# robert80203/HuPR-A-Benchmark-for-Human-Pose-Estimation-Using-Millimeter-Wave-Radar

Measured on AMD Instinct MI355X. Metric: radar frames/sec (FFT->heatmap fwd+bwd), higher is better.
Workload: dtype bf16

## Files before the change

### hupr-a-benchmark-for-human-pose-estimation-using-millimeter-wave-radar_amd/csrc/conv_halo256m_bf16.hip

```cpp
#include "conv_halo.h"

namespace hupr {

typedef float f32x4c __attribute__((ext_vector_type(4)));

template <int TD, int TH, int TW, int KD, int NCOT = 0, int NWN = 2, int KC = 64>
__global__ __launch_bounds__(512) void hupr_k_conv_halo256m_bf16(HaloArgs p) {
    constexpr int LDK = KC, BN = 32 * NWN, TS = KC == 64 ? 3 : 9, C8 = KC / 8, L2C8 = KC == 64 ? 3 : 2;
    static_assert(KC == 64 || (KC == 32 && KD == 3 && NWN == 2 && NCOT == 0), "32-channel rows: 3 x 3 x 3 taps, 64 output channels per tile");
    constexpr int HD = TD + KD - 1, HH = TH + 2, HW = TW + 2;
    static_assert(TD * TH * TW == 64 * (8 / NWN) && TH % 8 == 0 && TW % 8 == 0 && (KD == 1 || KD == 3) && (NWN == 2 || NCOT == 0),
                  "256 (512) voxels per tile, 8 x 8 per wave");
    constexpr int NVOX = HD * HH * HW;
    constexpr int T = 9 * KD, NSTAGE = KC == 64 ? 3 * KD : KD, NTAP = KC == 64 ? 6 : 9;
    constexpr bool FULLD = NWN == 1;
    constexpr int NVOXL = FULLD ? TD * HH * HW : NVOX, VOX0 = FULLD ? HH * HW : 0;
    constexpr int NH = (NVOXL * C8 + 511) / 512;
    constexpr int Y0 = NH < NTAP - 1 ? NH : NTAP - 1, Y1 = NH - (NTAP - 1) < 0 ? 0 : (NH - (NTAP - 1) > NTAP ? NTAP : NH - (NTAP - 1)),
                  Y2 = NH - (2 * NTAP - 1) < 0 ? 0 : (NH - (2 * NTAP - 1) > NTAP ? NTAP : NH - (2 * NTAP - 1));
    static_assert(NH <= NTAP * NSTAGE - 1 && NH <= 3 * NTAP - 1, "halo items must all be issued in front of the item's last barrier (and within three stages)");
    __shared__ __attribute__((aligned(16))) __bf16 Hs[(KC == 32 ? 2 : 1) * NVOX * LDK];
    __shared__ __attribute__((aligned(16))) __bf16 Bs[2][TS][BN * LDK];
    constexpr bool STATS = NCOT > 0 && KD == 3;
    constexpr bool SINGLE = STATS && TD == 2;
    f32x4c ssum[STATS ? NCOT : 1][2], ssq[STATS ? NCOT : 1][2];
    if constexpr (!SINGLE) {
#pragma unroll
        for (int ct = 0; ct < (STATS ? NCOT : 1); ++ct)
#pragma unroll
            for (int cg = 0; cg < 2; ++cg) { ssum[ct][cg] = (f32x4c){0.f, 0.f, 0.f, 0.f}; ssq[ct][cg] = (f32x4c){0.f, 0.f, 0.f, 0.f}; }
    }

    const int tid = threadIdx.x, lane = tid & 63, wave = tid >> 6;
    if (wave >= 4) __builtin_amdgcn_s_setprio(1);
    const int wm = NWN == 2 ? wave >> 1 : wave, wn = NWN == 2 ? wave & 1 : 0;
    constexpr int NBX = TW / 8, NBY = TH / 8;
    const int xw0 = 8 * (wm % NBX), yw0 = 8 * ((wm / NBX) % NBY), dzw = wm / (NBX * NBY);
    const int idx = lane & 15, kq = lane >> 4, yy = idx >> 3, wx = idx & 7;
    const int n_tiles = p.Bn * p.nd * p.nh * p.nw * p.n_co_tiles;

    const int wrow_ = NWN == 2 ? 8 * wave + (lane >> 3) : ((8 * wave + (lane >> 3)) & 31);
    const int wsrc_lane = (wrow_ * T * p.Ci + (((lane & 7) ^ (wrow_ >> 1)) & 7) * 8) * 2 +
                          (NWN == 2 ? 0 : (wave >> 2) * (3 * p.Ci * 2));
    constexpr int NDMA = NWN == 2 ? TS : 2, DMA_TAPS = NWN == 2 ? 1 : 2;
    const int wrow32_ = 16 * (wave & 3) + (lane >> 2);
    const int wsrc32_lane = (wrow32_ * T * p.Ci + (((lane & 3) ^ (((wrow32_ >> 3) & 1) << 1)) & 3) * 8) * 2;
    const u32x4 wrs = {(unsigned)(unsigned long)p.wp, (unsigned)((unsigned long)p.wp >> 32) & 0xffffu,
                       (unsigned)((long)p.Co * T * p.Ci * 2), 0x00020000u};
    const unsigned bs_lds = (unsigned)(unsigned long)(__attribute__((address_space(3))) void*)&Bs[0][0][0];
    const unsigned wdst_wave = __builtin_amdgcn_readfirstlane(bs_lds + wave * 1024);
#define HUPR_W_DMA(COT_, CH_, S_, PAR_)                                                                             \
    if constexpr (KC == 32) {                                                                                       \
        _Pragma("unroll") for (int j = 0; j < 5; ++j) {                                                             \
            if (j < 4 || wave < 4) {                                                                                \
                const int t9_ = 2 * j + (wave >> 2);                                  \
                const int wb32_ = (((COT_) * BN * T + (S_) * 9 + (t9_ % 3) * 3 + t9_ / 3) * p.Ci + (CH_) * KC) * 2 + wsrc32_lane; \
                unsigned keep_;                                                                                     \
                asm volatile("s_mov_b32 %0, m0\n\ts_mov_b32 m0, %1\n\ts_nop 0\n\tbuffer_load_dwordx4 %2, %3, 0 offen lds\n\t" \
                             "s_mov_b32 m0, %0"                                                                     \
                             : "=&s"(keep_)                                                                         \
                             : "s"(wdst_wave + (PAR_) * TS * (BN * LDK * 2) + j * 8192), "v"(wb32_), "s"(wrs)       \
                             : "memory");                                                                           \
            }                                                                                                       \
        }                                                                                                           \
    } else {                                                                                                        \
        const int wbase_ = (((COT_) * BN * T + ((S_) / 3) * 9 + ((S_) % 3)) * p.Ci + (CH_) * KC) * 2 + wsrc_lane;   \
        _Pragma("unroll") for (int j = 0; j < NDMA; ++j) {                                                          \
            if (NWN == 2 || j == 0 || wave < 4) {                                                                   \
                unsigned keep_;                                                                                     \
                asm volatile("s_mov_b32 %0, m0\n\ts_mov_b32 m0, %1\n\ts_nop 0\n\tbuffer_load_dwordx4 %2, %3, 0 offen lds\n\t" \
                             "s_mov_b32 m0, %0"                                                                     \
                             : "=&s"(keep_)                                                                         \
                             : "s"(NWN == 2 ? wdst_wave + ((PAR_) * TS + j) * (BN * LDK * 2)                        \
                                            : wdst_wave + (PAR_) * TS * (BN * LDK * 2) + j * 8192),                 \
                               "v"(NWN == 2 ? wbase_ + j * (3 * p.Ci * 2) : wbase_ + j * DMA_TAPS * (3 * p.Ci * 2)), "s"(wrs) \
                             : "memory");                                                                           \
            }                                                                                                       \
        }                                                                                                           \
    }

    u32x4 vb[NH];
    const __amdgpu_buffer_rsrc_t xrs = __builtin_amdgcn_make_buffer_rsrc(
        const_cast<void*>(p.x), 0, (int)((long)p.Bn * p.D * p.H * p.W * p.in_ld * 2), 0x00020000);
#define HUPR_HALO_ISSUE_ITEM(u, COND_, B_, D0_, H0_, W0_, C0_)                                                     \
    {                                                                                                               \
        const int it = tid + (u) * 512;                                                                             \
        const int vox = it >> L2C8, c8 = it & (C8 - 1);                                                             \
        const int hx = vox % HW;                                                                                    \
        const int t_ = vox / HW;                                                                                    \
        const int hy = t_ % HH, hz = t_ / HH;                                                                       \
        const int d = (D0_) + hz - (FULLD ? 0 : KD / 2), h = (H0_) + hy - 1, w = (W0_) + hx - 1;                    \
        const bool ok = (COND_) && it < NVOXL * C8 && (unsigned)d < (unsigned)p.D && (unsigned)h < (unsigned)p.H && \
                        (unsigned)w < (unsigned)p.W;                                                                \
        const int off = (((((B_) * p.D + d) * p.H + h) * p.W + w) * p.in_ld + (C0_) + c8 * 8) * 2;                  \
        const auto ld_ = __builtin_amdgcn_raw_buffer_load_b128(xrs, ok ? off : 0x7ffffff0, 0, 0);                  \
        vb[u] = (u32x4){ld_[0], ld_[1], ld_[2], ld_[3]};                                                            \
    }
#define HUPR_HALO_COMMIT()                                                                                          \
    _Pragma("unroll") for (int u = 0; u < NH; ++u) {                                                                \
        const int it = tid + u * 512;                                                                               \
        if (it < NVOXL * C8) {                                                                                      \
            const int vox = it >> L2C8, c8 = it & (C8 - 1);                                                         \
            const int hx = vox % HW;                                                                                \
            const int key_ = KC == 64 ? (((hx >> 1) & 3) << 1) : ((((vox / HW) % HH) & 1) << 1);                    \
            *reinterpret_cast<u32x4*>(&Hs[(vox + VOX0) * LDK + ((c8 ^ key_) << 3)]) = vb[u];                        \
        }                                                                                                           \
    }

    struct Pos { int cot, twi, thi, tdi, b, ch; };
    const int n_chunks = p.Ci / KC;
    const int per_wg = (n_tiles + gridDim.x - 1) / gridDim.x;
    const int wg_rank = (int)((blockIdx.x & 7) * (gridDim.x >> 3) + (blockIdx.x >> 3));
    const int t_begin = wg_rank * per_wg, t_end = min(n_tiles, t_begin + per_wg);
    if (STATS && p.stats) {
        if (t_begin >= t_end) {
            for (int c = tid; c < 2 * p.Co; c += 512) p.stats[(long)blockIdx.x * 2 * p.Co + c] = 0.0;
        }
    }
    if (t_begin >= t_end) return;
    Pos cur;
    {
        cur.cot = t_begin % p.n_co_tiles;
        int st = t_begin / p.n_co_tiles;
        cur.twi = st % p.nw; st /= p.nw;
        cur.thi = st % p.nh; st /= p.nh;
        cur.tdi = st % p.nd;
        cur.b = st / p.nd;
        cur.ch = 0;
    }
    const int n_items = (t_end - t_begin) * n_chunks;
    const int cot0 = cur.cot;

    int woff[2][2];
#pragma unroll
    for (int cg = 0; cg < 2; ++cg)
#pragma unroll
        for (int kk = 0; kk < 2; ++kk) {
            const int n = 32 * wn + 16 * cg + idx;
            woff[cg][kk] = KC == 64 ? n * LDK + (((4 * kk + kq) ^ ((n >> 1) & 7)) << 3) : n * LDK + ((kq ^ (((n >> 3) & 1) << 1)) << 3);
        }
    const int xlane = ((dzw * HH + yw0 + yy) * HW + xw0 + wx) * LDK;
#define HUPR_HALO_COMMIT1(u, HW_)                                                                                   \
    {                                                                                                               \
        const int it = tid + (u) * 512;                                                                             \
        if (it < NVOXL * C8) {                                                                                      \
            const int vox = it >> L2C8, c8 = it & (C8 - 1);                                                         \
            const int key_ = (((vox / HW) % HH) & 1) << 1;                                                          \
            *reinterpret_cast<u32x4*>(&Hs[(HW_) + (vox + VOX0) * LDK + ((c8 ^ key_) << 3)]) = vb[u];                \
        }                                                                                                           \
    }
#define HUPR_XF(ST_, RHO_, KK_)                                                                                     \
    (KC == 64 ? *reinterpret_cast<const bf16x8*>(&Hs[xlane + ((((ST_) / 3) * HH + (RHO_)) * HW + ((ST_) % 3)) * LDK + \
                    (((4 * (KK_) + kq) ^ ((((xw0 + wx + ((ST_) % 3)) >> 1) & 3) << 1)) << 3)])                      \
              : *reinterpret_cast<const bf16x8*>(&Hs[hrd + xlane + (((ST_) * HH + (RHO_)) * HW + (KK_)) * LDK +     \
                    ((kq ^ (((yy + (RHO_)) & 1) << 1)) << 3)]))
#define HUPR_WF(BUF_, KY_, CG_, KK_)                                                                                \
    (KC == 64 ? *reinterpret_cast<const bf16x8*>(&Bs[BUF_][KY_][woff[CG_][KK_]])                                    \
              : *reinterpret_cast<const bf16x8*>(&Bs[BUF_][3 * (KK_) + (KY_)][woff[CG_][0]]))

    f32x4c c[4][2];
    unsigned accP[4][2][2];
    __bf16* pP = nullptr;
    bool pend = false;
    constexpr bool RESPF = !STATS && TD != 2 && NWN == 2;
    const bool res_pf = RESPF && p.res != nullptr && (p.res_ld & 3) == 0 && !p.no_res_prefetch;
    constexpr bool BIASPF = KC == 32;
    const bool defer = (!p.bias || BIASPF) && (!p.res || res_pf) && (p.Co & 7) == 0 && (p.out_ld & 7) == 0;
    float biasv[BIASPF ? 2 : 1][4];
    bf16x4 resv[4][2];
    constexpr int NB = KC == 64 ? 2 : 3;
    bf16x8 xq[NB][4], x8, wq[NB][2];
#define HUPR_LOAD_TAP(ST_, TAU_, BUF_, WX_)                                                                         \
    {                                                                                                               \
        constexpr int kk_ = (TAU_) / 3, ky_ = (TAU_) % 3;                                                           \
        if ((WX_) & 1) {                                                                                            \
            wq[(TAU_) % NB][0] = HUPR_WF(BUF_, ky_, 0, kk_);                                                        \
            wq[(TAU_) % NB][1] = HUPR_WF(BUF_, ky_, 1, kk_);                                                        \
        }                                                                                                           \
        if ((WX_) & 2) {                                                                                            \
            if (ky_ == 0) { _Pragma("unroll") for (int vg = 0; vg < 4; ++vg) xq[kk_ % NB][vg] = HUPR_XF(ST_, 2 * vg, kk_); } \
            else if (ky_ == 1) { _Pragma("unroll") for (int vg = 0; vg < 4; ++vg) xq[(kk_ + 1) % NB][vg] = HUPR_XF(ST_, 2 * vg + 1, kk_); } \
            else { x8 = HUPR_XF(ST_, 8, kk_); }                                                                     \
        }                                                                                                           \
    }
#define HUPR_VMCNT_LGKM0(N_) __builtin_amdgcn_s_waitcnt(0x0070 | ((N_) & 15) | (((N_) >> 4) << 14))

    if constexpr (FULLD) {
        for (int i = tid; i < 2 * HH * HW * C8; i += 512) {
            const int pl = i / (HH * HW * C8), r = i - pl * (HH * HW * C8);
            *reinterpret_cast<u32x4*>(&Hs[pl * (HD - 1) * HH * HW * LDK + r * 8]) = (u32x4){0u, 0u, 0u, 0u};
        }
    }
    HUPR_W_DMA(cur.cot, cur.ch, 0, 0)
    HUPR_W_DMA(cur.cot, cur.ch, 1, 1)
#pragma unroll
    for (int u = 0; u < NH; ++u) HUPR_HALO_ISSUE_ITEM(u, true, cur.b, cur.tdi * TD, cur.thi * TH, cur.twi * TW, cur.ch * KC)
    [[maybe_unused]] int hrd = 0;
    if constexpr (KC == 32) {
#pragma unroll
        for (int u = 0; u < NH; ++u) HUPR_HALO_COMMIT1(u, 0)
    } else {
        HUPR_HALO_COMMIT()
    }
    __builtin_amdgcn_s_waitcnt(0x0F70);
    __syncthreads();
    HUPR_LOAD_TAP(0, 0, 0, 3)

    int g = 0;
    for (int q = 0; q < n_items; ++q) {
        const int b = cur.b, d0 = cur.tdi * TD, h0 = cur.thi * TH, w0 = cur.twi * TW, n0 = cur.cot * BN;
        const bool first_chunk = cur.ch == 0, last_chunk = cur.ch == n_chunks - 1;
        Pos nxt = cur;
        if (++nxt.ch == n_chunks) {
            nxt.ch = 0;
            if (++nxt.cot == p.n_co_tiles) {
                nxt.cot = 0;
                if (++nxt.twi == p.nw) {
                    nxt.twi = 0;
                    if (++nxt.thi == p.nh) {
                        nxt.thi = 0;
                        if (++nxt.tdi == p.nd) { nxt.tdi = 0; ++nxt.b; }
                    }
                }
            }
        }
        const bool has_next = q + 1 < n_items;
        if constexpr (KC == 32) hrd = (q & 1) * (NVOX * LDK);
        [[maybe_unused]] const int hwr = NVOX * LDK - hrd;
        if (first_chunk) {
#pragma unroll
            for (int vg = 0; vg < 4; ++vg)
#pragma unroll
                for (int cg = 0; cg < 2; ++cg) c[vg][cg] = (f32x4c){0.f, 0.f, 0.f, 0.f};
            if constexpr (BIASPF) {
                if (p.bias && defer) {
#pragma unroll
                    for (int cg = 0; cg < 2; ++cg)
#pragma unroll
                        for (int r = 0; r < 4; ++r) biasv[cg][r] = p.bias[n0 + 32 * wn + 16 * cg + 4 * kq + r];
                }
            }
        }
#pragma unroll
        for (int st_ = 0; st_ < NSTAGE; ++st_) {
            const int par = (g + st_) & 1;
#pragma unroll
            for (int tau = 0; tau < NTAP; ++tau) {
                const int kk = tau / 3, ky = tau % 3;
                if (tau == NTAP - 1) {
                    if (st_ == 0) { if (pend) { HUPR_VMCNT_LGKM0(Y0 + 4); } else { HUPR_VMCNT_LGKM0(Y0); } }
                    else if (st_ == 1) { HUPR_VMCNT_LGKM0(Y1); }
                    else if (st_ == 2) { HUPR_VMCNT_LGKM0(Y2); }
                    else { HUPR_VMCNT_LGKM0(0); }
                    __syncthreads();
                    if (st_ + 2 < NSTAGE) { HUPR_W_DMA(cur.cot, cur.ch, st_ + 2, par) }
                    else if (has_next) { HUPR_W_DMA(nxt.cot, nxt.ch, st_ + 2 - NSTAGE, par) }
                    if (KC == 64 && st_ == NSTAGE - 1 && has_next) { HUPR_HALO_COMMIT() }
                }
                if (tau == 0) { HUPR_LOAD_TAP(st_, 1, par, 3) }
                else if (tau == 1) { HUPR_LOAD_TAP(st_, 2, par, 3) }
                else if (tau == 2) { HUPR_LOAD_TAP(st_, 3, par, 3) }
                else if (tau == 3) { HUPR_LOAD_TAP(st_, 4, par, 3) }
                else if (tau == 4) { HUPR_LOAD_TAP(st_, 5, par, 3) }
                else if (NTAP == 9 && tau == 5) { if constexpr (NTAP == 9) { HUPR_LOAD_TAP(st_, 6, par, 3) } }
                else if (NTAP == 9 && tau == 6) { if constexpr (NTAP == 9) { HUPR_LOAD_TAP(st_, 7, par, 3) } }
                else if (NTAP == 9 && tau == 7) { if constexpr (NTAP == 9) { HUPR_LOAD_TAP(st_, 8, par, 3) } }
                else if (st_ + 1 < NSTAGE) { HUPR_LOAD_TAP((st_ + 1) % NSTAGE, 0, par ^ 1, 3) }
                else if (has_next) {
                    if constexpr (KC == 32) { const int hrd = hwr; HUPR_LOAD_TAP(0, 0, par ^ 1, 3) }
                    else { HUPR_LOAD_TAP(0, 0, par ^ 1, 1) }
                }
#pragma unroll
                for (int vg = 0; vg < 4; ++vg) {
                    const bf16x8 xf = ky == 0 ? xq[kk % NB][vg] : (ky == 1 ? xq[(kk + 1) % NB][vg] : (vg < 3 ? xq[kk % NB][vg + 1] : x8));
                    c[vg][0] = __builtin_amdgcn_mfma_f32_16x16x32_bf16(wq[tau % NB][0], xf, c[vg][0], 0, 0, 0);
                    c[vg][1] = __builtin_amdgcn_mfma_f32_16x16x32_bf16(wq[tau % NB][1], xf, c[vg][1], 0, 0, 0);
                }
                if (st_ == 0 && pend && tau < 4) {
                    const auto r0 = __builtin_amdgcn_permlane16_swap(accP[tau][0][0], accP[tau][1][0], false, false);
                    const auto r1 = __builtin_amdgcn_permlane16_swap(accP[tau][0][1], accP[tau][1][1], false, false);
                    *reinterpret_cast<u32x4*>(pP + (long)(2 * tau * p.W) * p.out_ld) = (u32x4){r0[0], r1[0], r0[1], r1[1]};
                }
                if (RESPF && st_ == NSTAGE - 1 && tau == 0) {
                    if (res_pf && last_chunk && defer) {
                        const long mr = (((long)b * p.D + d0 + dzw) * p.H + h0 + yw0 + yy) * p.W + w0 + xw0 + wx;
                        const int chr = n0 + 32 * wn + 4 * kq;
#pragma unroll
                        for (int vg = 0; vg < 4; ++vg)
#pragma unroll
                            for (int cg = 0; cg < 2; ++cg)
                                resv[vg][cg] = *reinterpret_cast<const bf16x4*>(static_cast<const __bf16*>(p.res) + (mr + 2 * vg * p.W) * p.res_ld +
                                                                                chr + 16 * cg);
                    }
                }
                if constexpr (KC == 32) {
                    if (st_ == NSTAGE - 1 && tau < NH && has_next) { HUPR_HALO_COMMIT1(tau, hwr) }
                }
                if (NTAP * st_ + tau < NH) {
                    HUPR_HALO_ISSUE_ITEM(NTAP * st_ + tau, has_next, nxt.b, nxt.tdi * TD, nxt.thi * TH, nxt.twi * TW, nxt.ch * KC)
                }
                __builtin_amdgcn_sched_group_barrier(0x100, 1, 0);
                __builtin_amdgcn_sched_group_barrier(0x008, 2, 0);
                __builtin_amdgcn_sched_group_barrier(0x100, 1, 0);
                __builtin_amdgcn_sched_group_barrier(0x008, 2, 0);
#pragma unroll
                for (int i_ = 0; i_ < 4; ++i_) {
                    __builtin_amdgcn_sched_group_barrier(0x100, 1, 0);
                    __builtin_amdgcn_sched_group_barrier(0x008, 1, 0);
                }
                __builtin_amdgcn_sched_barrier(0);
            }
            if (st_ == 0) pend = false;
        }
        g += NSTAGE;
        if (last_chunk) {
            const long m0 = (((long)b * p.D + d0 + dzw) * p.H + h0 + yw0 + yy) * p.W + w0 + xw0 + wx;
            const int ch0 = n0 + 32 * wn + 4 * kq;
            typedef __bf16 bf16x2 __attribute__((ext_vector_type(2)));
            if (defer && has_next) {
                if constexpr (BIASPF) {
                    if (p.bias) {
#pragma unroll
                        for (int vg = 0; vg < 4; ++vg)
#pragma unroll
                            for (int cg = 0; cg < 2; ++cg)
#pragma unroll
                                for (int r = 0; r < 4; ++r) c[vg][cg][r] += biasv[cg][r];
                    }
                }
                if (RESPF && res_pf) {
#pragma unroll
                    for (int vg = 0; vg < 4; ++vg)
#pragma unroll
                        for (int cg = 0; cg < 2; ++cg)
#pragma unroll
                            for (int r = 0; r < 4; ++r) c[vg][cg][r] += (float)resv[vg][cg][r];
                }
#pragma unroll
                for (int vg = 0; vg < 4; ++vg)
#pragma unroll
                    for (int cg = 0; cg < 2; ++cg) {
                        const bf16x2 lo = {(__bf16)c[vg][cg][0], (__bf16)c[vg][cg][1]}, hi = {(__bf16)c[vg][cg][2], (__bf16)c[vg][cg][3]};
                        accP[vg][cg][0] = __builtin_bit_cast(unsigned, lo);
                        accP[vg][cg][1] = __builtin_bit_cast(unsigned, hi);
                    }
                pP = static_cast<__bf16*>(p.y) + m0 * p.out_ld + n0 + 32 * wn + ((kq & 1) ? 16 + 4 * (kq - 1) : 4 * kq);
                pend = true;
            } else {
#pragma unroll
                for (int vg = 0; vg < 4; ++vg)
#pragma unroll
                    for (int cg = 0; cg < 2; ++cg) {
                        const long m = m0 + 2 * vg * p.W;
                        const int ch = ch0 + 16 * cg;
                        if (ch < p.Co) {
                            f32x4n v = {c[vg][cg][0], c[vg][cg][1], c[vg][cg][2], c[vg][cg][3]};
                            if (p.bias) v += (f32x4n){p.bias[ch], p.bias[ch + 1], p.bias[ch + 2], p.bias[ch + 3]};
                            if (p.res) {
                                const bf16x4 rv = *reinterpret_cast<const bf16x4*>(static_cast<const __bf16*>(p.res) + m * p.res_ld + ch);
                                v += (f32x4n){(float)rv[0], (float)rv[1], (float)rv[2], (float)rv[3]};
                            }
                            const bf16x4 o = {(__bf16)v[0], (__bf16)v[1], (__bf16)v[2], (__bf16)v[3]};
                            *reinterpret_cast<bf16x4*>(static_cast<__bf16*>(p.y) + m * p.out_ld + ch) = o;
                        }
                    }
            }
            if (STATS && p.stats) {
                int li = cur.cot - cot0;
                li += li < 0 ? p.n_co_tiles : 0;
                if constexpr (SINGLE) {
#pragma unroll
                    for (int cg = 0; cg < 2; ++cg) {
                        f32x4c sv = {0.f, 0.f, 0.f, 0.f}, qv = sv;
#pragma unroll
                        for (int vg = 0; vg < 4; ++vg)
#pragma unroll
                            for (int r = 0; r < 4; ++r) {
                                const float a = (float)(__bf16)c[vg][cg][r];
                                sv[r] += a;
                                qv[r] = fmaf(a, a, qv[r]);
                            }
                        ssum[0][cg] = sv;
                        ssq[0][cg] = qv;
                    }
                } else {
#pragma unroll
                    for (int ct = 0; ct < NCOT; ++ct)
                        if (NCOT == 1 || li == ct) {
#pragma unroll
                            for (int cg = 0; cg < 2; ++cg)
#pragma unroll
                                for (int vg = 0; vg < 4; ++vg)
#pragma unroll
                                    for (int r = 0; r < 4; ++r) {
                                        const float a = (float)(__bf16)c[vg][cg][r];
                                        ssum[ct][cg][r] += a;
                                        ssq[ct][cg][r] = fmaf(a, a, ssq[ct][cg][r]);
                                    }
                        }
                }
            }
        }
        if (KC == 64 && has_next) {
            __syncthreads();
            HUPR_LOAD_TAP(0, 0, g & 1, 2)
        }
        cur = nxt;
    }
    if (STATS && p.stats) {
        static_assert(NVOX * LDK * 2 >= 8 * 64 * 16 * 4, "the halo image must hold the reduction scratch");
        float (*St)[64][16] = reinterpret_cast<float (*)[64][16]>(Hs);
#pragma unroll
        for (int ct = 0; ct < NCOT; ++ct) {
            __syncthreads();
#pragma unroll
            for (int cg = 0; cg < 2; ++cg) {
                *reinterpret_cast<f32x4c*>(&St[wave][lane][4 * cg]) = ssum[ct][cg];
                *reinterpret_cast<f32x4c*>(&St[wave][lane][8 + 4 * cg]) = ssq[ct][cg];
            }
            __syncthreads();
            if (tid < 2 * BN) {
                const int k = tid >> 6, ch = tid & 63;
                const int wn_ = ch >> 5, cg = (ch >> 4) & 1, kq_ = (ch >> 2) & 3, r = ch & 3;
                double t = 0.0;
#pragma unroll
                for (int wm_ = 0; wm_ < 4; ++wm_)
#pragma unroll
                    for (int i = 0; i < 16; ++i) t += (double)St[2 * wm_ + wn_][16 * kq_ + i][8 * k + 4 * cg + r];
                p.stats[(long)blockIdx.x * 2 * p.Co + k * p.Co + 64 * ((cot0 + ct) % p.n_co_tiles) + ch] = t;
            }
        }
        if (tid < 2 * BN) {
            const int k = tid >> 6, ch = tid & 63;
            for (int ct = NCOT; ct < p.n_co_tiles; ++ct)
                p.stats[(long)blockIdx.x * 2 * p.Co + k * p.Co + 64 * ((cot0 + ct) % p.n_co_tiles) + ch] = 0.0;
        }
    }
#undef HUPR_W_DMA
#undef HUPR_HALO_ISSUE_ITEM
#undef HUPR_HALO_COMMIT
#undef HUPR_HALO_COMMIT1
#undef HUPR_XF
#undef HUPR_WF
#undef HUPR_LOAD_TAP
#undef HUPR_VMCNT_LGKM0
}

void launch_conv_halo256(const HaloArgs& a, int route, hipStream_t s) {
    const dim3 grid(kHalo256Grid), wg(512);
    switch (route) {
    case kRouteCi32: HUPR_LAUNCH((hupr_k_conv_halo256m_bf16<4, 8, 8, 3, 0, 2, 32>), grid, wg, 0, s, a); break;
    case kRouteCo32: HUPR_LAUNCH((hupr_k_conv_halo256m_bf16<8, 8, 8, 3, 0, 1>), grid, wg, 0, s, a); break;
    case kRoute1x16x16: HUPR_LAUNCH((hupr_k_conv_halo256m_bf16<1, 16, 16, 1>), grid, wg, 0, s, a); break;
    case kRouteStats4x8x8One: HUPR_LAUNCH((hupr_k_conv_halo256m_bf16<4, 8, 8, 3, 1>), grid, wg, 0, s, a); break;
    case kRouteStats4x8x8Two: HUPR_LAUNCH((hupr_k_conv_halo256m_bf16<4, 8, 8, 3, 2>), grid, wg, 0, s, a); break;
    case kRouteStats2x8x16: HUPR_LAUNCH((hupr_k_conv_halo256m_bf16<2, 8, 16, 3, 1>), grid, wg, 0, s, a); break;
    case kRoute4x8x8: HUPR_LAUNCH((hupr_k_conv_halo256m_bf16<4, 8, 8, 3>), grid, wg, 0, s, a); break;
    case kRoute2x8x16: HUPR_LAUNCH((hupr_k_conv_halo256m_bf16<2, 8, 16, 3>), grid, wg, 0, s, a); break;
    }
}

static int g_halo_tiles = 31;
void set_halo_tiles(int mask) { g_halo_tiles = mask & 31; }

static bool offsets_fit(const HaloArgs& a, int Bn) { return (long)Bn * a.D * a.H * a.W * a.in_ld * 2 < 0x7ffffff0L; }

bool conv_halo256_supported(const HaloArgs& a, int Bn, bool abf) {
    if (!abf || !(g_halo_tiles & 1)) return false;
    if (a.kd != 3 || a.D % 4 != 0 || a.H % 8 != 0 || a.W % 8 != 0 || a.Ci % 64 != 0 || a.Co % 64 != 0) return false;
    const long tiles = (long)Bn * (a.D / 4) * (a.H / 8) * (a.W / 8) * (a.Co / 64);
    if (tiles >= (1L << 31) || tiles < 256) return false;
    return offsets_fit(a, Bn);
}

bool conv_halo256_stats_ok(const HaloArgs& a, int Bn) {
    if (a.kd != 3 || a.Ci % 64 != 0 || a.Co % 64 != 0 || !offsets_fit(a, Bn)) return false;
    const int n = a.Co / 64;
    if (a.D % 4 == 0) {
        if (!conv_halo256_supported(a, Bn, true)) return false;
        if (n == 1) return true;
        const long tiles = (long)Bn * (a.D / 4) * (a.H / 8) * (a.W / 8) * n;
        const long per_wg = (tiles + kHalo256Grid - 1) / kHalo256Grid;
        return n <= 2 || per_wg == 1;
    }
    if (!(g_halo_tiles & 2) || a.D % 2 != 0 || a.H % 8 != 0 || a.W % 16 != 0) return false;
    return (long)Bn * (a.D / 2) * (a.H / 8) * (a.W / 16) * n == 256;
}

int conv_halo256_route(HaloArgs& a, int Bn, bool abf) {
    if (!abf || !offsets_fit(a, Bn)) return 0;
    if (a.Ci == 32) {
        if (!(g_halo_tiles & 16) || a.kd != 3 || a.D % 4 != 0 || a.H % 8 != 0 || a.W % 8 != 0 || a.Co % 64 != 0 || a.stats ||
            (a.in_ld & 7) || (long)a.Co * 27 * a.Ci * 2 >= 0x7ffffff0L)
            return 0;
        a.n_co_tiles = a.Co / 64;
        a.TD = 4; a.log2TW = 3;
        a.nd = a.D / 4; a.nh = a.H / 8; a.nw = a.W / 8;
        const long tiles_ = (long)Bn * a.nd * a.nh * a.nw * a.n_co_tiles;
        if (tiles_ < 256 || tiles_ >= (1L << 31)) return 0;
        return kRouteCi32;
    }
    if (a.Ci % 64 != 0) return 0;
    if (a.Co == 32) {
        if (!(g_halo_tiles & 8) || a.kd != 3 || a.D != 8 || a.H % 8 != 0 || a.W % 8 != 0 || a.stats || (a.out_ld & 7)) return 0;
        a.n_co_tiles = 1;
        a.TD = 8; a.log2TW = 3;
        a.nd = a.D / 8; a.nh = a.H / 8; a.nw = a.W / 8;
        const long tiles32 = (long)Bn * a.nd * a.nh * a.nw;
        if (tiles32 < 256 || tiles32 >= (1L << 31)) return 0;
        return kRouteCo32;
    }
    if (a.Co % 64 != 0) return 0;
    a.n_co_tiles = a.Co / 64;
    if (a.kd == 3 && a.D % 4 == 0) {
        if (!conv_halo256_supported(a, Bn, abf)) return 0;
        a.TD = 4; a.log2TW = 3;
        a.nd = a.D / 4; a.nh = a.H / 8; a.nw = a.W / 8;
    } else if (a.kd == 3) {
        if (!(g_halo_tiles & 2) || a.D % 2 != 0 || a.H % 8 != 0 || a.W % 16 != 0) return 0;
        a.TD = 2; a.log2TW = 4;
        a.nd = a.D / 2; a.nh = a.H / 8; a.nw = a.W / 16;
    } else {
        if (!(g_halo_tiles & 4) || a.kd != 1 || a.D != 1 || a.H % 16 != 0 || a.W % 16 != 0 || a.stats) return 0;
        a.TD = 1; a.log2TW = 4;
        a.nd = 1; a.nh = a.H / 16; a.nw = a.W / 16;
    }
    const long tiles = (long)Bn * a.nd * a.nh * a.nw * a.n_co_tiles;
    if (tiles < 256 || tiles >= (1L << 31)) return 0;
    if (a.TD == 1) return kRoute1x16x16;
    if (a.stats) {
        const long per_wg = (tiles + kHalo256Grid - 1) / kHalo256Grid;
        if (a.TD == 4) return (per_wg == 1 || a.n_co_tiles == 1) ? kRouteStats4x8x8One : kRouteStats4x8x8Two;
        return kRouteStats2x8x16;
    }
    return a.TD == 4 ? kRoute4x8x8 : kRoute2x8x16;
}

}
```

Measured before the change: 1735.

## Skip MFMA taps on zero depth-padding planes when the depth fits one tile

Adds a DSKIP template variant of the 3D halo conv kernel. When the whole depth fits in one tile (nd==1), it avoids loading and zero-filling the padding planes. Waves at the first or last depth slice then skip the kz=0 or kz=2 tap stages (LDS loads plus MFMAs), since those taps only see zero padding. Side work such as the pending stores, residual prefetch and halo issue is moved outside the skipped region so it still runs. The cost is wave-divergent work within a block, which can imbalance the barriers, and a reshuffled instruction schedule.

```diff
diff --git a/hupr-a-benchmark-for-human-pose-estimation-using-millimeter-wave-radar_amd/csrc/conv_halo256m_bf16.hip b/hupr-a-benchmark-for-human-pose-estimation-using-millimeter-wave-radar_amd/csrc/conv_halo256m_bf16.hip
--- a/hupr-a-benchmark-for-human-pose-estimation-using-millimeter-wave-radar_amd/csrc/conv_halo256m_bf16.hip
+++ b/hupr-a-benchmark-for-human-pose-estimation-using-millimeter-wave-radar_amd/csrc/conv_halo256m_bf16.hip
@@ -4,8 +4,9 @@
 
 typedef float f32x4c __attribute__((ext_vector_type(4)));
 
-template <int TD, int TH, int TW, int KD, int NCOT = 0, int NWN = 2, int KC = 64>
+template <int TD, int TH, int TW, int KD, int NCOT = 0, int NWN = 2, int KC = 64, int DSKIP = 0>
 __global__ __launch_bounds__(512) void hupr_k_conv_halo256m_bf16(HaloArgs p) {
+    static_assert(DSKIP == 0 || (DSKIP == 1 && KD == 3 && KC == 64 && NWN == 2), "depth-padding skip: 3 x 3 x 3 taps on 128-byte rows, 64 output channels per tile");
     constexpr int LDK = KC, BN = 32 * NWN, TS = KC == 64 ? 3 : 9, C8 = KC / 8, L2C8 = KC == 64 ? 3 : 2;
     static_assert(KC == 64 || (KC == 32 && KD == 3 && NWN == 2 && NCOT == 0), "32-channel rows: 3 x 3 x 3 taps, 64 output channels per tile");
     constexpr int HD = TD + KD - 1, HH = TH + 2, HW = TW + 2;
@@ -13,7 +14,7 @@
                   "256 (512) voxels per tile, 8 x 8 per wave");
     constexpr int NVOX = HD * HH * HW;
     constexpr int T = 9 * KD, NSTAGE = KC == 64 ? 3 * KD : KD, NTAP = KC == 64 ? 6 : 9;
-    constexpr bool FULLD = NWN == 1;
+    constexpr bool FULLD = NWN == 1 || DSKIP != 0;
     constexpr int NVOXL = FULLD ? TD * HH * HW : NVOX, VOX0 = FULLD ? HH * HW : 0;
     constexpr int NH = (NVOXL * C8 + 511) / 512;
     constexpr int Y0 = NH < NTAP - 1 ? NH : NTAP - 1, Y1 = NH - (NTAP - 1) < 0 ? 0 : (NH - (NTAP - 1) > NTAP ? NTAP : NH - (NTAP - 1)),
@@ -37,6 +38,8 @@
     constexpr int NBX = TW / 8, NBY = TH / 8;
     const int xw0 = 8 * (wm % NBX), yw0 = 8 * ((wm / NBX) % NBY), dzw = wm / (NBX * NBY);
     const int idx = lane & 15, kq = lane >> 4, yy = idx >> 3, wx = idx & 7;
+    [[maybe_unused]] const int dzs = __builtin_amdgcn_readfirstlane(dzw);
+#define HUPR_KZ_LIVE(KZ_) (DSKIP == 0 || (KZ_) == 1 ? true : ((KZ_) == 0 ? dzs != 0 : dzs != TD - 1))
     const int n_tiles = p.Bn * p.nd * p.nh * p.nw * p.n_co_tiles;
 
     const int wrow_ = NWN == 2 ? 8 * wave + (lane >> 3) : ((8 * wave + (lane >> 3)) & 31);
@@ -184,8 +187,36 @@
         }                                                                                                           \
     }
 #define HUPR_VMCNT_LGKM0(N_) __builtin_amdgcn_s_waitcnt(0x0070 | ((N_) & 15) | (((N_) >> 4) << 14))
-
-    if constexpr (FULLD) {
+#define HUPR_NEXT_STAGE_TAP0()                                                                                      \
+    if (st_ + 1 < NSTAGE) { if (live_next) { HUPR_LOAD_TAP((st_ + 1) % NSTAGE, 0, par ^ 1, 3) } }                    \
+    else if (has_next && live_next) {                                                                               \
+        if constexpr (KC == 32) { const int hrd = hwr; HUPR_LOAD_TAP(0, 0, par ^ 1, 3) }       \
+        else { HUPR_LOAD_TAP(0, 0, par ^ 1, 1) }                                                                    \
+    }
+#define HUPR_TAP_SIDE_WORK()                                                                                        \
+    if (st_ == 0 && pend && tau < 4) {                                                                              \
+        const auto r0 = __builtin_amdgcn_permlane16_swap(accP[tau][0][0], accP[tau][1][0], false, false);           \
+        const auto r1 = __builtin_amdgcn_permlane16_swap(accP[tau][0][1], accP[tau][1][1], false, false);           \
+        *reinterpret_cast<u32x4*>(pP + (long)(2 * tau * p.W) * p.out_ld) = (u32x4){r0[0], r1[0], r0[1], r1[1]};     \
+    }                                                                                                               \
+    if (RESPF && st_ == NSTAGE - 1 && tau == 0) {                                                                   \
+        if (res_pf && last_chunk && defer) {                                                                        \
+            const long mr = (((long)b * p.D + d0 + dzw) * p.H + h0 + yw0 + yy) * p.W + w0 + xw0 + wx;               \
+            const int chr = n0 + 32 * wn + 4 * kq;                                                                  \
+            _Pragma("unroll") for (int vg = 0; vg < 4; ++vg)                                                        \
+                _Pragma("unroll") for (int cg = 0; cg < 2; ++cg)                                                    \
+                    resv[vg][cg] = *reinterpret_cast<const bf16x4*>(static_cast<const __bf16*>(p.res) +             \
+                                                                    (mr + 2 * vg * p.W) * p.res_ld + chr + 16 * cg); \
+        }                                                                                                           \
+    }                                                                                                               \
+    if constexpr (KC == 32) {                                                                                       \
+        if (st_ == NSTAGE - 1 && tau < NH && has_next) { HUPR_HALO_COMMIT1(tau, hwr) }                              \
+    }                                                                                                               \
+    if (NTAP * st_ + tau < NH) {                                                                                    \
+        HUPR_HALO_ISSUE_ITEM(NTAP * st_ + tau, has_next, nxt.b, nxt.tdi * TD, nxt.thi * TH, nxt.twi * TW, nxt.ch * KC) \
+    }
+
+    if constexpr (FULLD && DSKIP == 0) {
         for (int i = tid; i < 2 * HH * HW * C8; i += 512) {
             const int pl = i / (HH * HW * C8), r = i - pl * (HH * HW * C8);
             *reinterpret_cast<u32x4*>(&Hs[pl * (HD - 1) * HH * HW * LDK + r * 8]) = (u32x4){0u, 0u, 0u, 0u};
@@ -204,7 +235,7 @@
     }
     __builtin_amdgcn_s_waitcnt(0x0F70);
     __syncthreads();
-    HUPR_LOAD_TAP(0, 0, 0, 3)
+    if (HUPR_KZ_LIVE(0)) { HUPR_LOAD_TAP(0, 0, 0, 3) }
 
     int g = 0;
     for (int q = 0; q < n_items; ++q) {
@@ -244,6 +275,9 @@
 #pragma unroll
         for (int st_ = 0; st_ < NSTAGE; ++st_) {
             const int par = (g + st_) & 1;
+            const int kz = KC == 64 ? st_ / 3 : st_, kzn = KC == 64 ? ((st_ + 1) % NSTAGE) / 3 : (st_ + 1) % NSTAGE;
+            const bool live = HUPR_KZ_LIVE(kz);
+            [[maybe_unused]] const bool live_next = HUPR_KZ_LIVE(kzn);
 #pragma unroll
             for (int tau = 0; tau < NTAP; ++tau) {
                 const int kk = tau / 3, ky = tau % 3;
@@ -257,58 +291,36 @@
                     else if (has_next) { HUPR_W_DMA(nxt.cot, nxt.ch, st_ + 2 - NSTAGE, par) }
                     if (KC == 64 && st_ == NSTAGE - 1 && has_next) { HUPR_HALO_COMMIT() }
                 }
-                if (tau == 0) { HUPR_LOAD_TAP(st_, 1, par, 3) }
-                else if (tau == 1) { HUPR_LOAD_TAP(st_, 2, par, 3) }
-                else if (tau == 2) { HUPR_LOAD_TAP(st_, 3, par, 3) }
-                else if (tau == 3) { HUPR_LOAD_TAP(st_, 4, par, 3) }
-                else if (tau == 4) { HUPR_LOAD_TAP(st_, 5, par, 3) }
-                else if (NTAP == 9 && tau == 5) { if constexpr (NTAP == 9) { HUPR_LOAD_TAP(st_, 6, par, 3) } }
-                else if (NTAP == 9 && tau == 6) { if constexpr (NTAP == 9) { HUPR_LOAD_TAP(st_, 7, par, 3) } }
-                else if (NTAP == 9 && tau == 7) { if constexpr (NTAP == 9) { HUPR_LOAD_TAP(st_, 8, par, 3) } }
-                else if (st_ + 1 < NSTAGE) { HUPR_LOAD_TAP((st_ + 1) % NSTAGE, 0, par ^ 1, 3) }
-                else if (has_next) {
-                    if constexpr (KC == 32) { const int hrd = hwr; HUPR_LOAD_TAP(0, 0, par ^ 1, 3) }
-                    else { HUPR_LOAD_TAP(0, 0, par ^ 1, 1) }
-                }
-#pragma unroll
-                for (int vg = 0; vg < 4; ++vg) {
-                    const bf16x8 xf = ky == 0 ? xq[kk % NB][vg] : (ky == 1 ? xq[(kk + 1) % NB][vg] : (vg < 3 ? xq[kk % NB][vg + 1] : x8));
-                    c[vg][0] = __builtin_amdgcn_mfma_f32_16x16x32_bf16(wq[tau % NB][0], xf, c[vg][0], 0, 0, 0);
-                    c[vg][1] = __builtin_amdgcn_mfma_f32_16x16x32_bf16(wq[tau % NB][1], xf, c[vg][1], 0, 0, 0);
-                }
-                if (st_ == 0 && pend && tau < 4) {
-                    const auto r0 = __builtin_amdgcn_permlane16_swap(accP[tau][0][0], accP[tau][1][0], false, false);
-                    const auto r1 = __builtin_amdgcn_permlane16_swap(accP[tau][0][1], accP[tau][1][1], false, false);
-                    *reinterpret_cast<u32x4*>(pP + (long)(2 * tau * p.W) * p.out_ld) = (u32x4){r0[0], r1[0], r0[1], r1[1]};
-                }
-                if (RESPF && st_ == NSTAGE - 1 && tau == 0) {
-                    if (res_pf && last_chunk && defer) {
-                        const long mr = (((long)b * p.D + d0 + dzw) * p.H + h0 + yw0 + yy) * p.W + w0 + xw0 + wx;
-                        const int chr = n0 + 32 * wn + 4 * kq;
-#pragma unroll
-                        for (int vg = 0; vg < 4; ++vg)
-#pragma unroll
-                            for (int cg = 0; cg < 2; ++cg)
-                                resv[vg][cg] = *reinterpret_cast<const bf16x4*>(static_cast<const __bf16*>(p.res) + (mr + 2 * vg * p.W) * p.res_ld +
-                                                                                chr + 16 * cg);
-                    }
-                }
-                if constexpr (KC == 32) {
-                    if (st_ == NSTAGE - 1 && tau < NH && has_next) { HUPR_HALO_COMMIT1(tau, hwr) }
-                }
-                if (NTAP * st_ + tau < NH) {
-                    HUPR_HALO_ISSUE_ITEM(NTAP * st_ + tau, has_next, nxt.b, nxt.tdi * TD, nxt.thi * TH, nxt.twi * TW, nxt.ch * KC)
-                }
-                __builtin_amdgcn_sched_group_barrier(0x100, 1, 0);
-                __builtin_amdgcn_sched_group_barrier(0x008, 2, 0);
-                __builtin_amdgcn_sched_group_barrier(0x100, 1, 0);
-                __builtin_amdgcn_sched_group_barrier(0x008, 2, 0);
-#pragma unroll
-                for (int i_ = 0; i_ < 4; ++i_) {
+                if (DSKIP != 0 && tau == NTAP - 1) { HUPR_NEXT_STAGE_TAP0() }
+                if (live) {
+                    if (tau == 0) { HUPR_LOAD_TAP(st_, 1, par, 3) }
+                    else if (tau == 1) { HUPR_LOAD_TAP(st_, 2, par, 3) }
+                    else if (tau == 2) { HUPR_LOAD_TAP(st_, 3, par, 3) }
+                    else if (tau == 3) { HUPR_LOAD_TAP(st_, 4, par, 3) }
+                    else if (tau == 4) { HUPR_LOAD_TAP(st_, 5, par, 3) }
+                    else if (NTAP == 9 && tau == 5) { if constexpr (NTAP == 9) { HUPR_LOAD_TAP(st_, 6, par, 3) } }
+                    else if (NTAP == 9 && tau == 6) { if constexpr (NTAP == 9) { HUPR_LOAD_TAP(st_, 7, par, 3) } }
+                    else if (NTAP == 9 && tau == 7) { if constexpr (NTAP == 9) { HUPR_LOAD_TAP(st_, 8, par, 3) } }
+                    else if (DSKIP == 0) { HUPR_NEXT_STAGE_TAP0() }
+#pragma unroll
+                    for (int vg = 0; vg < 4; ++vg) {
+                        const bf16x8 xf = ky == 0 ? xq[kk % NB][vg] : (ky == 1 ? xq[(kk + 1) % NB][vg] : (vg < 3 ? xq[kk % NB][vg + 1] : x8));
+                        c[vg][0] = __builtin_amdgcn_mfma_f32_16x16x32_bf16(wq[tau % NB][0], xf, c[vg][0], 0, 0, 0);
+                        c[vg][1] = __builtin_amdgcn_mfma_f32_16x16x32_bf16(wq[tau % NB][1], xf, c[vg][1], 0, 0, 0);
+                    }
+                    if constexpr (DSKIP == 0) { HUPR_TAP_SIDE_WORK() }
                     __builtin_amdgcn_sched_group_barrier(0x100, 1, 0);
-                    __builtin_amdgcn_sched_group_barrier(0x008, 1, 0);
-                }
-                __builtin_amdgcn_sched_barrier(0);
+                    __builtin_amdgcn_sched_group_barrier(0x008, 2, 0);
+                    __builtin_amdgcn_sched_group_barrier(0x100, 1, 0);
+                    __builtin_amdgcn_sched_group_barrier(0x008, 2, 0);
+#pragma unroll
+                    for (int i_ = 0; i_ < 4; ++i_) {
+                        __builtin_amdgcn_sched_group_barrier(0x100, 1, 0);
+                        __builtin_amdgcn_sched_group_barrier(0x008, 1, 0);
+                    }
+                    __builtin_amdgcn_sched_barrier(0);
+                }
+                if constexpr (DSKIP != 0) { HUPR_TAP_SIDE_WORK() }
             }
             if (st_ == 0) pend = false;
         }
@@ -403,7 +415,7 @@
         }
         if (KC == 64 && has_next) {
             __syncthreads();
-            HUPR_LOAD_TAP(0, 0, g & 1, 2)
+            if (HUPR_KZ_LIVE(0)) { HUPR_LOAD_TAP(0, 0, g & 1, 2) }
         }
         cur = nxt;
     }
@@ -444,20 +456,30 @@
 #undef HUPR_WF
 #undef HUPR_LOAD_TAP
 #undef HUPR_VMCNT_LGKM0
+#undef HUPR_KZ_LIVE
+#undef HUPR_NEXT_STAGE_TAP0
+#undef HUPR_TAP_SIDE_WORK
 }
+
+constexpr int kSkip4x8x8 = 1, kSkip2x8x16 = 1;
 
 void launch_conv_halo256(const HaloArgs& a, int route, hipStream_t s) {
     const dim3 grid(kHalo256Grid), wg(512);
+    const bool skip = a.nd == 1 && !(a.ablate & 8);
+#define HUPR_LAUNCH_SKIP(KEEP_, TD_, TH_, TW_, NCOT_)                                                                \
+    if ((KEEP_) && skip) HUPR_LAUNCH((hupr_k_conv_halo256m_bf16<TD_, TH_, TW_, 3, NCOT_, 2, 64, 1>), grid, wg, 0, s, a);           \
+    else HUPR_LAUNCH((hupr_k_conv_halo256m_bf16<TD_, TH_, TW_, 3, NCOT_>), grid, wg, 0, s, a)
     switch (route) {
     case kRouteCi32: HUPR_LAUNCH((hupr_k_conv_halo256m_bf16<4, 8, 8, 3, 0, 2, 32>), grid, wg, 0, s, a); break;
     case kRouteCo32: HUPR_LAUNCH((hupr_k_conv_halo256m_bf16<8, 8, 8, 3, 0, 1>), grid, wg, 0, s, a); break;
     case kRoute1x16x16: HUPR_LAUNCH((hupr_k_conv_halo256m_bf16<1, 16, 16, 1>), grid, wg, 0, s, a); break;
-    case kRouteStats4x8x8One: HUPR_LAUNCH((hupr_k_conv_halo256m_bf16<4, 8, 8, 3, 1>), grid, wg, 0, s, a); break;
-    case kRouteStats4x8x8Two: HUPR_LAUNCH((hupr_k_conv_halo256m_bf16<4, 8, 8, 3, 2>), grid, wg, 0, s, a); break;
-    case kRouteStats2x8x16: HUPR_LAUNCH((hupr_k_conv_halo256m_bf16<2, 8, 16, 3, 1>), grid, wg, 0, s, a); break;
-    case kRoute4x8x8: HUPR_LAUNCH((hupr_k_conv_halo256m_bf16<4, 8, 8, 3>), grid, wg, 0, s, a); break;
-    case kRoute2x8x16: HUPR_LAUNCH((hupr_k_conv_halo256m_bf16<2, 8, 16, 3>), grid, wg, 0, s, a); break;
-    }
+    case kRouteStats4x8x8One: HUPR_LAUNCH_SKIP(kSkip4x8x8, 4, 8, 8, 1); break;
+    case kRouteStats4x8x8Two: HUPR_LAUNCH_SKIP(kSkip4x8x8, 4, 8, 8, 2); break;
+    case kRouteStats2x8x16: HUPR_LAUNCH_SKIP(kSkip2x8x16, 2, 8, 16, 1); break;
+    case kRoute4x8x8: HUPR_LAUNCH_SKIP(kSkip4x8x8, 4, 8, 8, 0); break;
+    case kRoute2x8x16: HUPR_LAUNCH_SKIP(kSkip2x8x16, 2, 8, 16, 0); break;
+    }
+#undef HUPR_LAUNCH_SKIP
 }
 
 static int g_halo_tiles = 31;
```

After: 1752, median of 6. Within noise of the previous version (+1.0%).
